# kujason/monopsr

Measured on AMD Instinct MI355X. Metric: instance-crops/sec (fwd+Chamfer), higher is better.
Workload: dtype f32; 1 GPU; BASELINE cfg3: batch=256/GPU synthetic 48x48 crops -> ResNet-101 trunk(block3, os4) + squash/map-decoder/xyz + heads fwd, + 1024-pt nn_distance Chamfer fwd/bwd; batch_per_gpu=256, global_batch=256, points=1024, streams_per_gpu=1

## Files before the change

### include/monopsr_hip.h

```cpp
#ifndef MONOPSR_HIP_H
#define MONOPSR_HIP_H

#include <stddef.h>
#include <stdint.h>

#ifdef __cplusplus
extern "C" {
#endif

typedef void *mpsr_stream_t;
typedef void *mpsr_event_t;

enum {
    MPSR_OK = 0,
    MPSR_ERR_INVALID_ARG = 1,
    MPSR_ERR_HIP = 2,
    MPSR_ERR_WORKSPACE = 3,
    MPSR_ERR_UNSUPPORTED = 4
};

const char *mpsr_last_error(void);
int mpsr_abi_version(void);
uint32_t mpsr_crc32c(uint32_t crc, const void *data, size_t n);

// ... 27 lines not shown
int mpsr_match_cost_grad(int b, int n, int m, const float *xyz1, const float *xyz2, const float *match,
                         float *grad1, float *grad2, mpsr_stream_t stream);


int mpsr_crop_and_resize(const float *image, int nimg, int H, int W, int C, const float *boxes,
                         const int *box_ind, int nb, int ch, int cw, float extrapolation_value, float *out,
                         mpsr_stream_t stream);

int mpsr_resize_bilinear(const float *in, int B, int H, int W, int C, int OH, int OW, int align_corners,
                         float *out, mpsr_stream_t stream);

int mpsr_max_pool(const float *in, int B, int H, int W, int C, int k, int s, int pad_same, float *out,
                  mpsr_stream_t stream);


size_t mpsr_conv2d_scratch_floats(int B, int H, int W, int N);
int mpsr_conv2d_plan(int B, int H, int W, int C, int N, int KH, int KW, int dilation, int *kind,
                     double *executed_flops);
int mpsr_conv2d_nhwc_f32(const float *x, int B, int H, int W, int C, const float *w, const float *bias,
                         const float *residual, float *y, int N, int KH, int KW, int dilation, int relu,
                         int split_k, float *ws, size_t ws_floats, mpsr_stream_t stream);

enum { MPSR_CALL_MATH_INHERIT = 0, MPSR_CALL_MATH_FP32 = 1, MPSR_CALL_MATH_BF16X3 = 2 };
enum { MPSR_CALL_WINOGRAD_INHERIT = 0, MPSR_CALL_WINOGRAD_AUTO = 1, MPSR_CALL_WINOGRAD_OFF = 2,
       MPSR_CALL_WINOGRAD_ACCURATE = 3  };
typedef struct mpsr_conv_opts {
    int32_t math;
    int32_t winograd_policy;
} mpsr_conv_opts;
int mpsr_conv2d_nhwc_f32_ex(const float *x, int B, int H, int W, int C, const float *w, const float *bias,
// ... 304 lines not shown
```

### monopsr_amd/_lib.py

```python
import ctypes
import os

_HERE = os.path.dirname(os.path.abspath(__file__))
LIB_PATH = os.environ.get("MPSR_LIB_PATH") or os.path.join(_HERE, "libmonopsr_hip.so")
ABI_VERSION = 9

_lib = None


class MpsrError(RuntimeError):
    """A libmonopsr_hip.so call returned a non-zero status."""


class InvalidArgumentError(MpsrError, ValueError):
    """Shape/argument check failed -- the analogue of the tf.errors.InvalidArgumentError the reference's
    OP_REQUIRES checks raise (tf_nndistance.cpp:51-58, tf_approxmatch.cpp:152-165)."""


c_f = ctypes.c_void_p
c_i = ctypes.c_int
c_sz = ctypes.c_size_t


class Layer(ctypes.Structure):
# ... 59 lines not shown
    "mpsr_approx_match_temp_floats": (c_sz, [c_i, c_i, c_i]),
    "mpsr_emd_temp_floats": (c_sz, [c_i, c_i, c_i, c_i]),
    "mpsr_emd_loss_temp_floats": (c_sz, [c_i, c_i, c_i, c_i]),
    "mpsr_approx_match": (c_i, [c_i, c_i, c_i, c_f, c_f, c_f, c_f, c_sz, c_f]),
    "mpsr_approx_match_ex": (c_i, [c_i, c_i, c_i, c_f, c_f, c_f, c_f, c_sz, c_i, c_f]),
    "mpsr_emd_loss": (c_i, [c_i, c_i, c_i, c_f, c_f, c_f, c_f, c_f, c_f, c_sz, c_i, c_f]),
    "mpsr_match_cost": (c_i, [c_i, c_i, c_i, c_f, c_f, c_f, c_f, c_f]),
    "mpsr_match_cost_grad": (c_i, [c_i, c_i, c_i, c_f, c_f, c_f, c_f, c_f, c_f]),
    "mpsr_crop_and_resize": (c_i, [c_f, c_i, c_i, c_i, c_i, c_f, c_f, c_i, c_i, c_i, ctypes.c_float, c_f, c_f]),
    "mpsr_resize_bilinear": (c_i, [c_f, c_i, c_i, c_i, c_i, c_i, c_i, c_i, c_f, c_f]),
    "mpsr_max_pool": (c_i, [c_f, c_i, c_i, c_i, c_i, c_i, c_i, c_i, c_f, c_f]),
    "mpsr_conv2d_nhwc_f32": (c_i, [c_f, c_i, c_i, c_i, c_i, c_f, c_f, c_f, c_f, c_i, c_i, c_i, c_i, c_i, c_i, c_f,
                                   c_sz, c_f]),
    "mpsr_conv2d_nhwc_f32_ex": (c_i, [c_f, c_i, c_i, c_i, c_i, c_f, c_f, c_f, c_f, c_i, c_i, c_i, c_i, c_i, c_i, c_f,
                                      c_sz, ctypes.POINTER(ConvOpts), c_f]),
    "mpsr_conv2d_scratch_floats": (c_sz, [c_i, c_i, c_i, c_i]),
    "mpsr_conv2d_plan": (c_i, [c_i] * 8 + [ctypes.POINTER(c_i), ctypes.POINTER(ctypes.c_double)]),
    "mpsr_im2col_root": (c_i, [c_f, c_i, c_i, c_i, c_f, c_i, c_f]),
    "mpsr_conv2d_wgrad_f32": (c_i, [c_f, c_f, c_i, c_i, c_i, c_i, c_i, c_i, c_i, c_i, c_f, c_f, c_f]),
    "mpsr_conv2d_wgrad_scratch_floats": (c_sz, [c_i] * 8),
    "mpsr_conv2d_wgrad_ws_f32": (c_i, [c_f, c_f, c_i, c_i, c_i, c_i, c_i, c_i, c_i, c_i, c_f, c_f, c_f, c_sz, c_f]),
    "mpsr_conv2d_dgrad_pack": (c_i, [c_f, c_i, c_i, c_i, c_i, c_f, c_f]),
    "mpsr_dgrad_pack_table_bytes": (c_sz, [ctypes.POINTER(PackJob), c_i]),
    "mpsr_dgrad_pack_table_build": (c_i, [ctypes.POINTER(PackJob), c_i, ctypes.c_void_p,
                                          ctypes.POINTER(ctypes.c_longlong)]),
    "mpsr_conv2d_dgrad_pack_batch": (c_i, [c_f, ctypes.c_longlong, c_f]),
    "mpsr_act_bias_grad": (c_i, [c_f, c_f, c_f, c_f, ctypes.c_longlong, c_i, c_f]),
    "mpsr_bias_grad": (c_i, [c_f, ctypes.c_longlong, c_i, c_f, c_f]),
    "mpsr_relu_grad": (c_i, [c_f, c_f, c_f, ctypes.c_longlong, c_f]),
    "mpsr_conv2d_relu_masked_f32": (c_i, [c_f, c_i, c_i, c_i, c_i, c_f, c_f, c_f, c_i, c_i, c_i, c_i, c_f, c_sz, c_f]),
# ... 154 lines not shown
```

### monopsr_amd/csrc/conv_mfma.hip

```cpp
#include <atomic>
#include <mutex>
#include <type_traits>

#include "common.h"

namespace {

using f32x16 = __attribute__((ext_vector_type(16))) float;
using f32x4 = __attribute__((ext_vector_type(4))) float;
using bf16x4 = __attribute__((ext_vector_type(4))) __bf16;
using bf16x8 = __attribute__((ext_vector_type(8))) __bf16;

constexpr int MATH_FP32 = 0, MATH_BF16X3 = 1;

constexpr int BK = 32;
constexpr int LDS_STRIDE = BK + 4;
constexpr int MAX_CLS = 9;

using mpsr::FastDiv;
using mpsr::fdiv;
using mpsr::make_fastdiv;

struct PixelClass {
    int y0, h, x0, w;
// ... 935 lines not shown
size_t winograd4_split_floats(int B, int H, int W, int N);
extern std::atomic<int> g_wino4_split;
size_t winograd3_scratch_floats(int C, int N);
bool winograd3_applies(int H, int W, int C, int dilation);
double winograd3_executed_flops(int B, int H, int C, int N, int dilation);
int winograd3_form(int B, int H, int W, int C, int N, int dilation);
int conv3x3_winograd3(const float *x, int B, int H, int W, int C, const float *w, const float *bias, int relu,
                      float *y, int N, int dilation, float *ws, size_t ws_floats, hipStream_t s,
                      const float *mask = nullptr);

bool pointwise_applies(long long M, int K, int N);
int pointwise_override();
int conv1x1_pointwise(const float *x, long long M, int K, const float *w, const float *bias, const float *residual,
                      int relu, float *y, int N, hipStream_t s);

bool thin_input_conv_applies(int B, int H, int W, int C, int N, int KH, int KW, int dilation);
int thin_input_conv(const float *x, int B, int H, int W, const float *w, const float *bias, int relu, float *y, int N,
                    hipStream_t s);

bool fc_rows_applies(long long M, int K, int N);
bool fc_rows_split_applies(long long M, int K, int N, const float *bias, const float *y, const float *ws, size_t ws_floats);
int fc_rows_split(const float *x, long long M, int K, const float *w, const float *bias, int relu, float *y, int N,
                  float *ws, hipStream_t s);
int fc_rows(const float *x, long long M, int K, const float *w, const float *bias, const float *residual, int relu,
            float *y, int N, hipStream_t s);

bool conv2d_takes_fc_rows(int H, int W, long long M, int C, int N, int KH, int KW, int split_k)
{
    const int pw = pointwise_override();
    return H == 1 && W == 1 && KH == 1 && KW == 1 && split_k <= 1 && pw != 0 && cur_math() == MATH_FP32 &&
           g_tile_override.load() < 0 && g_sched_override.load() < 0 && fc_rows_applies(M, C, N);
}

bool conv2d_takes_pointwise(long long M, int C, int N, int KH, int KW, int split_k)
{
    const int pw = pointwise_override();
    if (KH != 1 || KW != 1 || split_k > 1 || pw == 0 || cur_math() != MATH_FP32 || g_tile_override.load() >= 0 ||
        !pointwise_applies(M, C, N))
        return false;
    if (pw > 0) return true;
    if (g_sched_override.load() >= 0 || g_class_override.load() >= 0) return false;
    const long long tiles = ((M + 95) / 96) * ((N + 127) / 128);
    return split_k == 0 && N % 128 == 0 && tiles >= 512;
}

size_t conv_auto_split_floats() { return (size_t)1536 * 64 * 64; }
size_t conv_scratch_floats(long long M, int N)
{
    const size_t slabs = (size_t)1024 * 2 * 96 * 128;
    const size_t counters = (size_t)((M + 63) / 64 + 9) * (size_t)((N + 31) / 32);
    return slabs + counters;
}

int g_auto_split_target = 768;
constexpr int g_auto_split_enough = 768;
constexpr int g_auto_split_min_ksteps = 4;

int auto_split_k(int M, int N, int ksteps, const float *ws, size_t ws_floats)
// ... 79 lines not shown
    const long long M64 = (long long)B * H * W;
    MPSR_REQUIRE(M64 * C * 4 < 0xfffffff0LL && (long long)N * KH * KW * C * 4 < 0xfffffff0LL && M64 < 0x7fffffffLL,
                 "conv2d: tensor exceeds the 4 GiB addressable by one launch; split the batch");
    if (KH == 3 && KW == 3 && dilation == 1 && N <= 4 && C % 32 == 0 && !residual && split_k <= 1 &&
        g_tile_override.load() < 0 && ((uintptr_t)w & 3) == 0)
        return conv3x3_narrow(x, B, H, W, C, w, bias, relu, y, N, stream, 0);
    if (!residual && split_k <= 1 && g_tile_override.load() < 0 && cur_math() == MATH_FP32 &&
        thin_input_conv_applies(B, H, W, C, N, KH, KW, dilation))
        return thin_input_conv(x, B, H, W, w, bias, relu, y, N, stream);
    if (!residual && conv2d_takes_winograd3(B, H, W, C, N, KH, KW, dilation, split_k, ws, ws_floats))
        return conv3x3_winograd3(x, B, H, W, C, w, bias, relu, y, N, dilation, ws, ws_floats, stream);
    {
        const int wc = conv2d_winograd_choice(B, H, W, C, N, KH, KW, dilation, residual != nullptr, split_k, ws, ws_floats);
        if (wc == 2) return conv3x3_winograd4(x, B, H, W, C, w, bias, relu, y, N, ws, ws_floats, stream, 0, 0, nullptr, 0);
        if (wc == 1) return conv3x3_winograd(x, B, H, W, C, w, bias, relu, y, N, ws, ws_floats, stream, dilation);
    }
    if (conv2d_takes_pointwise(M64, C, N, KH, KW, split_k))
        return conv1x1_pointwise(x, M64, C, w, bias, residual, relu, y, N, stream);
    if (conv2d_takes_fc_rows(H, W, M64, C, N, KH, KW, split_k))
        return fc_rows(x, M64, C, w, bias, residual, relu, y, N, stream);
    if (H == 1 && W == 1 && KH == 1 && KW == 1 && !residual && split_k == 0 && pointwise_override() != 0 &&
        cur_math() == MATH_FP32 && g_tile_override.load() < 0 && g_sched_override.load() < 0 &&
        fc_rows_split_applies(M64, C, N, bias, y, ws, ws_floats))
        return fc_rows_split(x, M64, C, w, bias, relu, y, N, ws, stream);
    ConvParams p;
    p.x = x; p.w = w; p.bias = bias; p.residual = residual; p.y = y; p.ws = ws; p.ws_floats = ws ? ws_floats : 0;
    p.M = (int)M64; p.H = H; p.W = W; p.C = C; p.N = N; p.KH = KH; p.KW = KW; p.dil = dilation; p.relu = relu;
    p.xbytes = (unsigned)(M64 * C * 4);
    p.wbytes = (unsigned)((long long)N * KH * KW * C * 4);
    p.cblocks = ceil_div(C, BK);
// ... 125 lines not shown
    if (wc == 1) {
        *kind = 1;
        *executed_flops = 2.0 * (double)B * (H / 2) * (W / 2) * 16.0 * C * N;
        return MPSR_OK;
    }
    if (KH == 3 && KW == 3 && dilation == 1 && N <= 4 && C % 32 == 0) {
        *kind = 2;
        *executed_flops = 2.0 * M * 9.0 * C * N;
        return MPSR_OK;
    }
    if (mpsr::thin_input_conv_applies(B, H, W, C, N, KH, KW, dilation)) {
        *kind = 2;
        *executed_flops = 2.0 * M * 9.0 * C * N;
        return MPSR_OK;
    }
    if (mpsr::conv2d_takes_pointwise((long long)B * H * W, C, N, KH, KW, 0)) {
        *kind = 5;
        *executed_flops = 2.0 * M * C * N;
        return MPSR_OK;
    }
    if (mpsr::conv2d_takes_fc_rows(H, W, (long long)B * H * W, C, N, KH, KW, 0)) {
        *kind = 6;
        *executed_flops = 2.0 * M * C * N;
        return MPSR_OK;
    }
    *kind = 0;
    double taps = (double)KH * KW * H * W;
    if (KH == 3 && KW == 3 && dilation > 1 && H >= 2 * dilation && W >= 2 * dilation) {
        const double ty = 3.0 * H - 2.0 * dilation, tx = 3.0 * W - 2.0 * dilation;
        taps = ty * tx;
// ... 3 lines not shown
}

extern "C" size_t mpsr_conv2d_scratch_floats(int B, int H, int W, int N)
{
    if (B <= 0 || H <= 0 || W <= 0 || N <= 0) return 0;
    size_t n = mpsr::conv_scratch_floats((long long)B * H * W, N);
    if (mpsr::g_wino4_split.load() != 0 && (long long)B * H * W >= 65536 && N % 128 == 0 && H % 4 == 0 && W % 4 == 0)
        n += mpsr::winograd4_split_floats(B, H, W, N) + 64;
    return n;
}

extern "C" int mpsr_conv2d_nhwc_f32(const float *x, int B, int H, int W, int C, const float *w, const float *bias,
                                    const float *residual, float *y, int N, int KH, int KW, int dilation, int relu,
                                    int split_k, float *ws, size_t ws_floats, mpsr_stream_t stream)
{
    return mpsr::conv2d(x, B, H, W, C, w, bias, residual, y, N, KH, KW, dilation, relu, split_k, ws, ws_floats,
                        mpsr::as_stream(stream));
}

extern "C" int mpsr_conv2d_nhwc_f32_ex(const float *x, int B, int H, int W, int C, const float *w, const float *bias,
                                       const float *residual, float *y, int N, int KH, int KW, int dilation, int relu,
                                       int split_k, float *ws, size_t ws_floats, const mpsr_conv_opts *opts,
                                       mpsr_stream_t stream)
{
    if (opts) {
        MPSR_REQUIRE(opts->math >= 0 && opts->math <= MPSR_CALL_MATH_BF16X3, "conv2d: unknown opts.math %d", opts->math);
        MPSR_REQUIRE(opts->winograd_policy >= 0 && opts->winograd_policy <= MPSR_CALL_WINOGRAD_ACCURATE,
                     "conv2d: unknown opts.winograd_policy %d", opts->winograd_policy);
    }
    mpsr::CallOptsGuard guard(opts ? opts->math : 0, opts ? opts->winograd_policy : 0);
    return mpsr::conv2d(x, B, H, W, C, w, bias, residual, y, N, KH, KW, dilation, relu, split_k, ws, ws_floats,
                        mpsr::as_stream(stream));
}

extern "C" int mpsr_conv2d_relu_masked_f32(const float *x, int B, int H, int W, int C, const float *w, const float *mask,
                                           float *y, int N, int KH, int KW, int dilation, float *ws, size_t ws_floats,
                                           mpsr_stream_t stream)
{
    MPSR_REQUIRE(mask, "conv2d_relu_masked: null mask");
    hipStream_t s = mpsr::as_stream(stream);
    if (B > 0 && x && w && y && mpsr::conv2d_takes_winograd3(B, H, W, C, N, KH, KW, dilation, 0, ws, ws_floats))
        return mpsr::conv3x3_winograd3(x, B, H, W, C, w, nullptr, 0, y, N, dilation, ws, ws_floats, s, mask);
    if (int rc = mpsr::conv2d(x, B, H, W, C, w, nullptr, nullptr, y, N, KH, KW, dilation, 0, 0, ws, ws_floats, s)) return rc;
    return mpsr_relu_grad(y, mask, y, (long long)B * H * W * N, stream);
}
// ... 192 lines not shown
```

### monopsr_amd/csrc/network.hip

```cpp
#include <atomic>
#include <vector>

#include "common.h"
#include "wino3_filter.h"

namespace mpsr {
int conv2d(const float *x, int B, int H, int W, int C, const float *w, const float *bias, const float *residual,
           float *y, int N, int KH, int KW, int dilation, int relu, int split_k, float *ws, size_t ws_floats,
           hipStream_t stream);
size_t conv_scratch_floats(long long M, int N);
bool conv2d_takes_winograd4(int B, int H, int W, int C, int N, const float *ws, size_t ws_floats);
int conv3x3_winograd4(const float *x, int B, int H, int W, int C, const float *w, const float *bias, int relu,
                      float *y, int N, float *ws, size_t ws_floats, hipStream_t s, int in_c8, int out_c8, float *part,
                      size_t part_floats);
size_t winograd4_split_floats(int B, int H, int W, int N);
extern std::atomic<int> g_wino4_split;
int winograd3_filter_form(int B, int H, int W, int C, int N, int dilation);
bool conv2d_takes_winograd3(int B, int H, int W, int C, int N, int KH, int KW, int dilation, int split_k, const float *ws,
                            size_t ws_floats);
bool conv2d_takes_pointwise(long long M, int C, int N, int KH, int KW, int split_k);
int conv3x3_narrow(const float *x, int B, int H, int W, int C, const float *w, const float *bias, int relu, float *y,
                   int N, hipStream_t s, int in_c8);
bool conv3x3_narrow_takes_mfma(const float *x, int B, int H, int W, int C, int N, const float *w);
int conv2d_winograd_choice(int B, int H, int W, int C, int N, int KH, int KW, int dilation, bool residual, int split_k,
                           const float *ws, size_t ws_floats);
int resize_bilinear_c8(const float *in, int B, int H, int W, int C, int OH, int OW, int align_corners, float *out,
                       hipStream_t s);
bool upconv_applies(int B, int h, int w, int C, int OH, int OW, int N, int align_corners);
size_t upconv_z_floats(long long Msrc, int N);
size_t upconv_weight_floats(int C, int N);
int conv3x3_upsampled(const float *x, int B, int h, int w, int C, int OH, int OW, int align_corners, const float *g,
                      const float *bias, int relu, float *y, int N, int out_c8, float *z, size_t z_floats, float *ws,
                      size_t ws_floats, hipStream_t s);
}

// ... 28 lines not shown
int run_layer(const float *blob, const mpsr_layer &L, const float *x, int B, int H, int W, const float *residual,
              float *y, int split_k, float *ws, size_t ws_floats, hipStream_t s)
{
    return mpsr::conv2d(x, B, H, W, L.cin, blob + L.w_off, L.b_off >= 0 ? blob + L.b_off : nullptr, residual, y, L.cout,
                        L.kh, L.kw, L.dilation, L.relu, split_k, ws, ws_floats, s);
}

constexpr int kTrunkUnits[3] = {3, 4, 23};

inline size_t cache_floats_of(const mpsr_layer &L)
{
    if (L.kh != 3 || L.kw != 3) return 0;
    return mpsr::align_up((size_t)(L.dilation > 1 ? 25 : 36) * (size_t)L.cout * (size_t)L.cin, 64);
}

struct FilterCache {
    float *base = nullptr;
    size_t floats = 0, used = 0;
    bool valid = false;
    int *tags = nullptr;
    explicit FilterCache(const mpsr_net_opts *o)
    {
        if (o && o->filter_cache && o->filter_cache_floats) {
            base = o->filter_cache;
            floats = o->filter_cache_floats;
            valid = o->filter_cache_valid != 0;
            tags = o->filter_cache_tags;
        }
    }
    float *take(const mpsr_layer &L)
    {
        const size_t need = cache_floats_of(L);
        if (!base || need == 0) return nullptr;
        float *r = used + need <= floats ? base + used : nullptr;
        used += need;
        return r;
    }
    void offer(const float *w, float *slice, const mpsr_layer &L, int layer_index) const
    {
        mpsr::g_filter_cache_slot = mpsr::FilterCacheSlot();
        if (slice) {
            mpsr::g_filter_cache_slot.w = w;
            mpsr::g_filter_cache_slot.u = slice;
            mpsr::g_filter_cache_slot.floats = cache_floats_of(L);
            mpsr::g_filter_cache_slot.ready = valid;
            mpsr::g_filter_cache_slot.tag = tags ? tags + layer_index : nullptr;
        }
    }
};

struct TrunkDims {
// ... 13 lines not shown


extern "C" size_t mpsr_trunk_workspace_bytes(int B, int H, int W)
{
    if (B <= 0 || H <= 0 || W <= 0) return 0;
    const TrunkDims d = trunk_dims(H, W);
    const size_t Mr = (size_t)B * d.OH * d.OW, Mp = (size_t)B * d.PH * d.PW;
    return fbytes(Mr * 160) + fbytes(Mr * 64) + fbytes(Mp * 64) + 3 * fbytes(Mp * 1024) + 2 * fbytes(Mp * 256) +
           fbytes(mpsr::conv_scratch_floats((long long)(Mr > Mp ? Mr : Mp), 1024));
}

extern "C" size_t mpsr_filter_cache_floats(const mpsr_layer *layers, int n_layers)
{
    size_t n = 0;
    if (layers)
        for (int i = 0; i < n_layers; ++i) n += cache_floats_of(layers[i]);
    return n;
}

extern "C" int mpsr_trunk_fwd(const float *img, int B, int H, int W, const float *blob, const mpsr_layer *layers,
                              int n_layers, float *out, void *workspace, size_t workspace_bytes, mpsr_stream_t stream)
{
    return mpsr_trunk_fwd_ex(img, B, H, W, blob, layers, n_layers, out, workspace, workspace_bytes, nullptr, stream);
}

extern "C" int mpsr_trunk_fwd_ex(const float *img, int B, int H, int W, const float *blob, const mpsr_layer *layers,
                                 int n_layers, float *out, void *workspace, size_t workspace_bytes,
                                 const mpsr_net_opts *opts, mpsr_stream_t stream)
{
    MPSR_REQUIRE(B >= 0 && H >= 7 && W >= 7, "trunk_fwd: bad input shape (B=%d H=%d W=%d)", B, H, W);
    if (opts) {
// ... 27 lines not shown
    float *sk = ar.floats(skn);
    if (!ar.ok)
        return mpsr::fail(MPSR_ERR_WORKSPACE, "trunk_fwd: workspace %zu bytes too small (see mpsr_trunk_workspace_bytes)",
                          workspace_bytes);

    int rc;
    struct TailJobGuard {
        ~TailJobGuard()
        {
            mpsr::g_filter_tail_job = mpsr::FilterTailJob();
            mpsr::g_filter_tail_done = mpsr::FilterTailJob();
            mpsr::g_filter_cache_slot = mpsr::FilterCacheSlot();
        }
    } tail_job_guard;
    FilterCache cache(opts);
    if ((rc = mpsr_im2col_root(img, B, H, W, cols, root.cin, stream))) return rc;
    if ((rc = run_layer(blob, root, cols, B, d.OH, d.OW, nullptr, rootout, 0, sk, skn, s))) return rc;
    if ((rc = mpsr_max_pool(rootout, B, d.OH, d.OW, root.cout, 3, 2, 1, pooled, stream))) return rc;

    const float *cur = pooled;
    int cur_c = root.cout;
    int li = 1;
    for (int blk = 0; blk < 3; ++blk) {
        for (int u = 0; u < kTrunkUnits[blk]; ++u) {
            const bool last = (blk == 2 && u == kTrunkUnits[blk] - 1);
            const float *residual = cur;
            if (u == 0) {
                const mpsr_layer &S = layers[li++];
                MPSR_REQUIRE(S.kh == 1 && S.cin == cur_c && !S.relu, "trunk_fwd: record %d is not a shortcut", li - 1);
                if ((rc = run_layer(blob, S, cur, B, d.PH, d.PW, nullptr, scut, 0, sk, skn, s))) return rc;
                residual = scut;
            }
            const mpsr_layer &c1 = layers[li], &c2 = layers[li + 1], &c3 = layers[li + 2];
            li += 3;
            MPSR_REQUIRE(c1.kh == 1 && c1.cin == cur_c && c2.kh == 3 && c2.cin == c1.cout && c3.kh == 1 &&
                             c3.cin == c2.cout && (u == 0 || c3.cout == cur_c),
                         "trunk_fwd: records %d..%d do not form a bottleneck unit", li - 3, li - 1);
            float *dst = last ? out : (cur == ping ? pong : ping);
            float *uslice = cache.take(c2);
            const int c2i = (int)(&c2 - layers);
            const int fform = mpsr::winograd3_filter_form(B, d.PH, d.PW, c2.cin, c2.cout, c2.dilation);
            const bool cached_u = uslice && cache.valid && (!cache.tags || cache.tags[c2i] == fform);
            if (!cached_u &&
                mpsr::conv2d_takes_pointwise((long long)B * d.PH * d.PW, c1.cin, c1.cout, 1, 1, 0) &&
                mpsr::conv2d_takes_winograd3(B, d.PH, d.PW, c2.cin, c2.cout, c2.kh, c2.kw, c2.dilation, 0, sk, skn)) {
                mpsr::g_filter_tail_job.w = blob + c2.w_off;
                mpsr::g_filter_tail_job.u = uslice ? uslice : sk;
                mpsr::g_filter_tail_job.N = c2.cout;
                mpsr::g_filter_tail_job.C = c2.cin;
                mpsr::g_filter_tail_job.form = fform == mpsr::FILTER_FORM_WINO3Z ? 1 : 0;
            }
            if ((rc = run_layer(blob, c1, cur, B, d.PH, d.PW, nullptr, t1, 0, sk, skn, s))) return rc;
            mpsr::g_filter_tail_job = mpsr::FilterTailJob();
            cache.offer(blob + c2.w_off, uslice, c2, c2i);
            rc = run_layer(blob, c2, t1, B, d.PH, d.PW, nullptr, t2, 0, sk, skn, s);
            mpsr::g_filter_cache_slot = mpsr::FilterCacheSlot();
            if (rc) return rc;
            if ((rc = run_layer(blob, c3, t2, B, d.PH, d.PW, residual, dst, 0, sk, skn, s))) return rc;
            cur = dst;
            cur_c = c3.cout;
        }
    }
    return MPSR_OK;
}


namespace {
struct DecoderChoice {
    bool c8, up1, up2, xyz_c8;
};
DecoderChoice decoder_choice(int B, int fh, int fw, int mh, int mw, const mpsr_layer *L, const float *blob, bool feat_map,
                             bool xyz_map, const float *sk, size_t skn)
{
// ... 106 lines not shown
    size_t partn = 0;
    float *partb = nullptr;
    if (ar.ok && mpsr::g_wino4_split.load() != 0 && c2 % 128 == 0 && c3 % 128 == 0 && hh % 4 == 0 && hw % 4 == 0 && mh % 4 == 0 && mw % 4 == 0) {
        const size_t a1 = mpsr::winograd4_split_floats(B, hh, hw, c2), a2 = mpsr::winograd4_split_floats(B, mh, mw, c3);
        partn = (a1 > a2 ? a1 : a2) + 64;
        partb = ar.floats(partn);
        if (!ar.ok) {
            ar.ok = true;
            partb = nullptr;
            partn = 0;
        }
    }
    if (!ar.ok)
        return mpsr::fail(MPSR_ERR_WORKSPACE, "squash_decoder_fwd: workspace %zu bytes too small", workspace_bytes);
    int rc;
    if ((rc = run_layer(blob, L[0], crop_feat, B, fh, fw, nullptr, part, 0, sk, skn, s))) return rc;
    if ((rc = run_layer(blob, L[1], full_feat, B, fh, fw, part, sq, 0, sk, skn, s))) return rc;
    if ((rc = mpsr_max_pool(sq, B, fh, fw, csq, 2, 2, 0, feat_box3d, stream))) return rc;
    if (opts && opts->ready_event) MPSR_CHECK_HIP(hipEventRecord(reinterpret_cast<hipEvent_t>(opts->ready_event), s));
    struct SlotGuard {
        ~SlotGuard() { mpsr::g_filter_cache_slot = mpsr::FilterCacheSlot(); }
    } slot_guard;
    FilterCache cache(opts);
    const DecoderChoice ch = decoder_choice(B, fh, fw, mh, mw, L, blob, feat_map != nullptr, xyz_map != nullptr, sk, skn);
    const bool xyz_c8 = ch.xyz_c8, up1 = ch.up1, up2 = ch.up2, c8 = ch.c8;
    if (c8) {
        auto wino = [&](const mpsr_layer &Lr, const float *x, int H, int W, float *y, int in_c8, int out_c8) {
            cache.offer(blob + Lr.w_off, cache.take(Lr), Lr, (int)(&Lr - L));
            return mpsr::conv3x3_winograd4(x, B, H, W, Lr.cin, blob + Lr.w_off, Lr.b_off >= 0 ? blob + Lr.b_off : nullptr,
                                           Lr.relu, y, Lr.cout, sk, skn, s, in_c8, out_c8, partb, partn);
        };
        auto upconv = [&](const mpsr_layer &Lr, const float *x, int h, int w, int H, int W, float *y, float *z, size_t zn) {
            cache.offer(blob + Lr.w_off, cache.take(Lr), Lr, (int)(&Lr - L));
            return mpsr::conv3x3_upsampled(x, B, h, w, Lr.cin, H, W, 1, blob + Lr.w_off,
                                           Lr.b_off >= 0 ? blob + Lr.b_off : nullptr, Lr.relu, y, Lr.cout, 1, z, zn, sk,
                                           skn, s);
        };
        if (up1) {
// ... 252 lines not shown
```

### monopsr_amd/csrc/wino3_filter.h

```cpp
#pragma once
#include <hip/hip_runtime.h>

namespace mpsr {
namespace f3f {
constexpr int KC = 8, NP = 25;
}

__device__ __forceinline__ void wino3_filter_one(const float *__restrict__ w, int N, int C, float *__restrict__ u, long long i)
{
    const int n = (int)(i / C), c = (int)(i - (long long)n * C);
    double g[3][3];
#pragma unroll
    for (int ky = 0; ky < 3; ++ky)
#pragma unroll
        for (int kx = 0; kx < 3; ++kx) g[ky][kx] = (double)w[(size_t)n * 9 * C + (size_t)(ky * 3 + kx) * C + c];
    auto gcol = [](double a, double b, double c2, double *o) {
        o[0] = a / 2.0;
        o[1] = (a + b + c2) / 2.0;
        o[2] = (a - b + c2) / 6.0;
        o[3] = a / 6.0 + b / 3.0 + c2 * (2.0 / 3.0);
        o[4] = c2;
    };
    double t[5][3];
#pragma unroll
// ... 59 lines not shown
extern thread_local FilterTailJob g_filter_tail_done;

struct FilterCacheSlot {
    const float *w = nullptr;
    float *u = nullptr;
    size_t floats = 0;
    bool ready = false;
    int *tag = nullptr;
    bool holds(int kind)
    {
        const bool ok = ready && (!tag || *tag == kind);
        if (tag) *tag = kind;
        return ok;
    }
};
enum { FILTER_FORM_WINO4 = 1, FILTER_FORM_WINO3 = 2, FILTER_FORM_UPCONV = 3, FILTER_FORM_WINO3Z = 4, FILTER_FORM_WINO2 = 5 };
extern thread_local FilterCacheSlot g_filter_cache_slot;
}
```

### monopsr_amd/csrc/winograd3.hip

```cpp
#include <atomic>
#include <type_traits>

#include "common.h"
#include "wino3_filter.h"
#include "wino3_transforms.h"

namespace {

using f32x16 = __attribute__((ext_vector_type(16))) float;

namespace f3 {
constexpr int MT = 32, NT = 64, KC = 8, NP = 25;
constexpr int APOS = MT * KC;
constexpr int ABUF = NP * APOS;
constexpr int MEXF = NP * 16 * NT;
constexpr int LDSF = MEXF > 2 * ABUF ? MEXF : 2 * ABUF;
constexpr unsigned OOB = 0x80000000u;
}

struct Wino3Params {
    const float *x, *u, *bias;
    float *y;
    int B, H, W, C, N, dil, T;
    int th;
// ... 343 lines not shown
int winograd3_form(int B, int H, int W, int C, int N, int dilation)
{
    const int th = H / (3 * dilation);
    if (th != 1 || !winograd3w_applies(B, H, W, C, N, dilation)) return 0;
    const int form = g_wino3_form.load();
    return (form >= 0 && form <= 2) ? form : 2;
}
int winograd3_filter_form(int B, int H, int W, int C, int N, int dilation)
{
    return winograd3_form(B, H, W, C, N, dilation) == 2 ? FILTER_FORM_WINO3Z : FILTER_FORM_WINO3;
}

thread_local FilterTailJob g_filter_tail_job;
thread_local FilterTailJob g_filter_tail_done;
thread_local FilterCacheSlot g_filter_cache_slot;

size_t winograd3_scratch_floats(int C, int N) { return (size_t)f3::NP * N * C; }

bool winograd3_applies(int H, int W, int C, int dilation)
{
    return dilation >= 1 && H == W && H % (3 * dilation) == 0 && H / (3 * dilation) <= 16 && C % 16 == 0 && C >= 16;
}

long long winograd3_tiles(int B, int H, int dilation)
{
    const int th = H / (3 * dilation);
    return (long long)B * dilation * dilation * th * th;
}
double winograd3_executed_flops(int B, int H, int C, int N, int dilation)
{
// ... 74 lines not shown
```

Baseline: 19280 crops/s.

## Add Strassen 7-multiply pointwise conv kernel with cached filter planes

Adds a 1x1 convolution kernel that applies one level of Strassen over 2x2 blocks of the K and N dimensions. It builds seven combined activation planes in LDS and seven precomputed weight planes, so it issues 7 MFMA products where the plain GEMM issues 8. The weight planes are cached in the trunk and squash filter caches, and half the output quadrants are swapped between waves through LDS before the epilogue. It is on by default when the tile count is large, at the cost of extra adds, LDS traffic, cache memory and looser fp32 accuracy.

```diff
diff --git a/include/monopsr_hip.h b/include/monopsr_hip.h
--- a/include/monopsr_hip.h
+++ b/include/monopsr_hip.h
@@ -65,6 +65,7 @@
                   mpsr_stream_t stream);
 
 
+int mpsr_debug_set_pointwise_strassen(int mode);
 size_t mpsr_conv2d_scratch_floats(int B, int H, int W, int N);
 int mpsr_conv2d_plan(int B, int H, int W, int C, int N, int KH, int KW, int dilation, int *kind,
                      double *executed_flops);
diff --git a/monopsr_amd/_lib.py b/monopsr_amd/_lib.py
--- a/monopsr_amd/_lib.py
+++ b/monopsr_amd/_lib.py
@@ -97,6 +97,7 @@
                                    c_sz, c_f]),
     "mpsr_conv2d_nhwc_f32_ex": (c_i, [c_f, c_i, c_i, c_i, c_i, c_f, c_f, c_f, c_f, c_i, c_i, c_i, c_i, c_i, c_i, c_f,
                                       c_sz, ctypes.POINTER(ConvOpts), c_f]),
+    "mpsr_debug_set_pointwise_strassen": (c_i, [c_i]),
     "mpsr_conv2d_scratch_floats": (c_sz, [c_i, c_i, c_i, c_i]),
     "mpsr_conv2d_plan": (c_i, [c_i] * 8 + [ctypes.POINTER(c_i), ctypes.POINTER(ctypes.c_double)]),
     "mpsr_im2col_root": (c_i, [c_f, c_i, c_i, c_i, c_f, c_i, c_f]),
diff --git a/monopsr_amd/csrc/conv_mfma.hip b/monopsr_amd/csrc/conv_mfma.hip
--- a/monopsr_amd/csrc/conv_mfma.hip
+++ b/monopsr_amd/csrc/conv_mfma.hip
@@ -3,6 +3,7 @@
 #include <type_traits>
 
 #include "common.h"
+#include "wino3_filter.h"
 
 namespace {
 
@@ -973,6 +974,13 @@
 int conv1x1_pointwise(const float *x, long long M, int K, const float *w, const float *bias, const float *residual,
                       int relu, float *y, int N, hipStream_t s);
 
+int pointwise_s7_mode();
+bool pointwise_s7_applies(long long M, int K, int N);
+size_t pointwise_s7_plane_floats(int K, int N);
+int pointwise_s7_fill(const float *w, int K, int N, float *planes, hipStream_t s);
+int conv1x1_pointwise_s7(const float *x, long long M, int K, const float *planes, const float *bias, const float *residual,
+                         int relu, float *y, int N, hipStream_t s);
+
 bool thin_input_conv_applies(int B, int H, int W, int C, int N, int KH, int KW, int dilation);
 int thin_input_conv(const float *x, int B, int H, int W, const float *w, const float *bias, int relu, float *y, int N,
                     hipStream_t s);
@@ -1001,6 +1009,18 @@
     if (g_sched_override.load() >= 0 || g_class_override.load() >= 0) return false;
     const long long tiles = ((M + 95) / 96) * ((N + 127) / 128);
     return split_k == 0 && N % 128 == 0 && tiles >= 512;
+}
+
+bool conv2d_takes_pointwise_s7(long long M, int C, int N, int KH, int KW, int split_k)
+{
+    const int mode = pointwise_s7_mode(), pw = pointwise_override();
+    if (mode == 0 || KH != 1 || KW != 1 || split_k > 1 || pw == 0 || cur_math() != MATH_FP32 || g_tile_override.load() >= 0 ||
+        !pointwise_s7_applies(M, C, N))
+        return false;
+    if (mode == 2) return true;
+    if (pw > 0 || !conv2d_takes_pointwise(M, C, N, KH, KW, split_k)) return false;
+    const long long tiles = ((M + 63) / 64) * (N / 128);
+    return tiles >= 1024;
 }
 
 size_t conv_auto_split_floats() { return (size_t)1536 * 64 * 64; }
@@ -1110,6 +1130,23 @@
         const int wc = conv2d_winograd_choice(B, H, W, C, N, KH, KW, dilation, residual != nullptr, split_k, ws, ws_floats);
         if (wc == 2) return conv3x3_winograd4(x, B, H, W, C, w, bias, relu, y, N, ws, ws_floats, stream, 0, 0, nullptr, 0);
         if (wc == 1) return conv3x3_winograd(x, B, H, W, C, w, bias, relu, y, N, ws, ws_floats, stream, dilation);
+    }
+    if (conv2d_takes_pointwise_s7(M64, C, N, KH, KW, split_k)) {
+        const size_t need = pointwise_s7_plane_floats(C, N);
+        float *planes = nullptr;
+        bool ready = false;
+        if (g_filter_cache_slot.w == w && g_filter_cache_slot.u && g_filter_cache_slot.floats >= need) {
+            planes = g_filter_cache_slot.u;
+            ready = g_filter_cache_slot.holds(FILTER_FORM_PW_S7);
+            g_filter_cache_slot = FilterCacheSlot();
+        } else if (g_conv2d_single_layer && ws && ws_floats >= need && ((uintptr_t)ws & 15) == 0) {
+            planes = ws;
+        }
+        if (planes) {
+            if (!ready)
+                if (int rc = pointwise_s7_fill(w, C, N, planes, stream)) return rc;
+            return conv1x1_pointwise_s7(x, M64, C, planes, bias, residual, relu, y, N, stream);
+        }
     }
     if (conv2d_takes_pointwise(M64, C, N, KH, KW, split_k))
         return conv1x1_pointwise(x, M64, C, w, bias, residual, relu, y, N, stream);
@@ -1265,6 +1302,11 @@
         *executed_flops = 2.0 * M * 9.0 * C * N;
         return MPSR_OK;
     }
+    if (mpsr::conv2d_takes_pointwise_s7((long long)B * H * W, C, N, KH, KW, 0)) {
+        *kind = 5;
+        *executed_flops = 2.0 * M * C * N * 7.0 / 8.0;
+        return MPSR_OK;
+    }
     if (mpsr::conv2d_takes_pointwise((long long)B * H * W, C, N, KH, KW, 0)) {
         *kind = 5;
         *executed_flops = 2.0 * M * C * N;
@@ -1298,6 +1340,10 @@
                                     const float *residual, float *y, int N, int KH, int KW, int dilation, int relu,
                                     int split_k, float *ws, size_t ws_floats, mpsr_stream_t stream)
 {
+    struct SingleLayer {
+        SingleLayer() { mpsr::g_conv2d_single_layer = true; }
+        ~SingleLayer() { mpsr::g_conv2d_single_layer = false; }
+    } single_layer;
     return mpsr::conv2d(x, B, H, W, C, w, bias, residual, y, N, KH, KW, dilation, relu, split_k, ws, ws_floats,
                         mpsr::as_stream(stream));
 }
@@ -1313,6 +1359,10 @@
                      "conv2d: unknown opts.winograd_policy %d", opts->winograd_policy);
     }
     mpsr::CallOptsGuard guard(opts ? opts->math : 0, opts ? opts->winograd_policy : 0);
+    struct SingleLayer {
+        SingleLayer() { mpsr::g_conv2d_single_layer = true; }
+        ~SingleLayer() { mpsr::g_conv2d_single_layer = false; }
+    } single_layer;
     return mpsr::conv2d(x, B, H, W, C, w, bias, residual, y, N, KH, KW, dilation, relu, split_k, ws, ws_floats,
                         mpsr::as_stream(stream));
 }
diff --git a/monopsr_amd/csrc/network.hip b/monopsr_amd/csrc/network.hip
--- a/monopsr_amd/csrc/network.hip
+++ b/monopsr_amd/csrc/network.hip
@@ -19,6 +19,7 @@
 bool conv2d_takes_winograd3(int B, int H, int W, int C, int N, int KH, int KW, int dilation, int split_k, const float *ws,
                             size_t ws_floats);
 bool conv2d_takes_pointwise(long long M, int C, int N, int KH, int KW, int split_k);
+bool conv2d_takes_pointwise_s7(long long M, int C, int N, int KH, int KW, int split_k);
 int conv3x3_narrow(const float *x, int B, int H, int W, int C, const float *w, const float *bias, int relu, float *y,
                    int N, hipStream_t s, int in_c8);
 bool conv3x3_narrow_takes_mfma(const float *x, int B, int H, int W, int C, int N, const float *w);
@@ -77,6 +78,12 @@
     return mpsr::align_up((size_t)(L.dilation > 1 ? 25 : 36) * (size_t)L.cout * (size_t)L.cin, 64);
 }
 
+inline size_t cache_floats_of_1x1(const mpsr_layer &L)
+{
+    if (L.kh != 1 || L.kw != 1 || L.cin < 256 || L.cin > 2048 || L.cin % 64 || L.cout % 128 || L.cout > 2048) return 0;
+    return mpsr::align_up((size_t)7 * (size_t)L.cout * (size_t)L.cin / 4, 64);
+}
+
 struct FilterCache {
     float *base = nullptr;
     size_t floats = 0, used = 0;
@@ -98,6 +105,26 @@
         float *r = used + need <= floats ? base + used : nullptr;
         used += need;
         return r;
+    }
+    size_t base_1x1 = 0, used_1x1 = 0;
+    void layers(const mpsr_layer *L, int n)
+    {
+        for (int i = 0; i < n; ++i) base_1x1 += cache_floats_of(L[i]);
+    }
+    void offer_1x1(const float *w, const mpsr_layer &L, int layer_index, long long M)
+    {
+        const size_t need = cache_floats_of_1x1(L);
+        if (!base || need == 0) return;
+        float *slice = base_1x1 + used_1x1 + need <= floats ? base + base_1x1 + used_1x1 : nullptr;
+        used_1x1 += need;
+        mpsr::g_filter_cache_slot = mpsr::FilterCacheSlot();
+        if (slice && mpsr::conv2d_takes_pointwise_s7(M, L.cin, L.cout, 1, 1, 0)) {
+            mpsr::g_filter_cache_slot.w = w;
+            mpsr::g_filter_cache_slot.u = slice;
+            mpsr::g_filter_cache_slot.floats = need;
+            mpsr::g_filter_cache_slot.ready = valid;
+            mpsr::g_filter_cache_slot.tag = tags ? tags + layer_index : nullptr;
+        }
     }
     void offer(const float *w, float *slice, const mpsr_layer &L, int layer_index) const
     {
@@ -141,7 +168,7 @@
 {
     size_t n = 0;
     if (layers)
-        for (int i = 0; i < n_layers; ++i) n += cache_floats_of(layers[i]);
+        for (int i = 0; i < n_layers; ++i) n += cache_floats_of(layers[i]) + cache_floats_of_1x1(layers[i]);
     return n;
 }
 
@@ -199,6 +226,13 @@
         }
     } tail_job_guard;
     FilterCache cache(opts);
+    cache.layers(layers, n_layers);
+    auto run_1x1 = [&](const mpsr_layer &L1, const float *x, const float *res, float *y) {
+        cache.offer_1x1(blob + L1.w_off, L1, (int)(&L1 - layers), (long long)Mp);
+        const int r = run_layer(blob, L1, x, B, d.PH, d.PW, res, y, 0, sk, skn, s);
+        mpsr::g_filter_cache_slot = mpsr::FilterCacheSlot();
+        return r;
+    };
     if ((rc = mpsr_im2col_root(img, B, H, W, cols, root.cin, stream))) return rc;
     if ((rc = run_layer(blob, root, cols, B, d.OH, d.OW, nullptr, rootout, 0, sk, skn, s))) return rc;
     if ((rc = mpsr_max_pool(rootout, B, d.OH, d.OW, root.cout, 3, 2, 1, pooled, stream))) return rc;
@@ -213,7 +247,7 @@
             if (u == 0) {
                 const mpsr_layer &S = layers[li++];
                 MPSR_REQUIRE(S.kh == 1 && S.cin == cur_c && !S.relu, "trunk_fwd: record %d is not a shortcut", li - 1);
-                if ((rc = run_layer(blob, S, cur, B, d.PH, d.PW, nullptr, scut, 0, sk, skn, s))) return rc;
+                if ((rc = run_1x1(S, cur, nullptr, scut))) return rc;
                 residual = scut;
             }
             const mpsr_layer &c1 = layers[li], &c2 = layers[li + 1], &c3 = layers[li + 2];
@@ -235,13 +269,13 @@
                 mpsr::g_filter_tail_job.C = c2.cin;
                 mpsr::g_filter_tail_job.form = fform == mpsr::FILTER_FORM_WINO3Z ? 1 : 0;
             }
-            if ((rc = run_layer(blob, c1, cur, B, d.PH, d.PW, nullptr, t1, 0, sk, skn, s))) return rc;
+            if ((rc = run_1x1(c1, cur, nullptr, t1))) return rc;
             mpsr::g_filter_tail_job = mpsr::FilterTailJob();
             cache.offer(blob + c2.w_off, uslice, c2, c2i);
             rc = run_layer(blob, c2, t1, B, d.PH, d.PW, nullptr, t2, 0, sk, skn, s);
             mpsr::g_filter_cache_slot = mpsr::FilterCacheSlot();
             if (rc) return rc;
-            if ((rc = run_layer(blob, c3, t2, B, d.PH, d.PW, residual, dst, 0, sk, skn, s))) return rc;
+            if ((rc = run_1x1(c3, t2, residual, dst))) return rc;
             cur = dst;
             cur_c = c3.cout;
         }
@@ -378,14 +412,18 @@
     if (!ar.ok)
         return mpsr::fail(MPSR_ERR_WORKSPACE, "squash_decoder_fwd: workspace %zu bytes too small", workspace_bytes);
     int rc;
-    if ((rc = run_layer(blob, L[0], crop_feat, B, fh, fw, nullptr, part, 0, sk, skn, s))) return rc;
-    if ((rc = run_layer(blob, L[1], full_feat, B, fh, fw, part, sq, 0, sk, skn, s))) return rc;
-    if ((rc = mpsr_max_pool(sq, B, fh, fw, csq, 2, 2, 0, feat_box3d, stream))) return rc;
-    if (opts && opts->ready_event) MPSR_CHECK_HIP(hipEventRecord(reinterpret_cast<hipEvent_t>(opts->ready_event), s));
     struct SlotGuard {
         ~SlotGuard() { mpsr::g_filter_cache_slot = mpsr::FilterCacheSlot(); }
     } slot_guard;
     FilterCache cache(opts);
+    cache.layers(L, n_layers);
+    cache.offer_1x1(blob + L[0].w_off, L[0], 0, (long long)B * fh * fw);
+    if ((rc = run_layer(blob, L[0], crop_feat, B, fh, fw, nullptr, part, 0, sk, skn, s))) return rc;
+    cache.offer_1x1(blob + L[1].w_off, L[1], 1, (long long)B * fh * fw);
+    if ((rc = run_layer(blob, L[1], full_feat, B, fh, fw, part, sq, 0, sk, skn, s))) return rc;
+    mpsr::g_filter_cache_slot = mpsr::FilterCacheSlot();
+    if ((rc = mpsr_max_pool(sq, B, fh, fw, csq, 2, 2, 0, feat_box3d, stream))) return rc;
+    if (opts && opts->ready_event) MPSR_CHECK_HIP(hipEventRecord(reinterpret_cast<hipEvent_t>(opts->ready_event), s));
     const DecoderChoice ch = decoder_choice(B, fh, fw, mh, mw, L, blob, feat_map != nullptr, xyz_map != nullptr, sk, skn);
     const bool xyz_c8 = ch.xyz_c8, up1 = ch.up1, up2 = ch.up2, c8 = ch.c8;
     if (c8) {
diff --git a/monopsr_amd/csrc/pointwise_s7.hip b/monopsr_amd/csrc/pointwise_s7.hip
--- /dev/null
+++ b/monopsr_amd/csrc/pointwise_s7.hip
@@ -0,0 +1,281 @@
+#include <atomic>
+
+#include "common.h"
+#include "wino3_filter.h"
+
+namespace {
+
+using f32x16 = __attribute__((ext_vector_type(16))) float;
+
+namespace s7 {
+constexpr int ROWS = 64, COLS = 128, KS = 32;
+constexpr int PLANE_B = 32 * (KS / 2) * 4;
+constexpr int STAGE_B = 7 * PLANE_B;
+constexpr int XCH_OFF = 2 * STAGE_B;
+constexpr int XCH_B = 4 * 2 * 16 * 64 * 4;
+constexpr int LDS_B = XCH_OFF + XCH_B;
+constexpr unsigned OOB = 0x80000000u;
+}
+
+struct S7Params {
+    const float *x, *planes, *bias, *residual;
+    float *y;
+    int M, N, K, relu;
+    int cblocks, ntiles;
+    unsigned xbytes, pbytes, ybytes;
+    const float *fw;
+    float *fu;
+    int fN, fC, fform;
+};
+
+template <bool RES>
+__global__ __launch_bounds__(256) __attribute__((amdgpu_waves_per_eu(2, 2))) void pw_conv_kernel_s7(const S7Params p)
+{
+    using namespace s7;
+    extern __shared__ __attribute__((aligned(16))) char lds[];
+    const int tid = threadIdx.x, lane = tid & 63;
+    const int wave = __builtin_amdgcn_readfirstlane(tid >> 6);
+    const int wc = wave & 1, kh = wave >> 1;
+    const int nst = p.K / KS;
+    constexpr int STORE_AUX = RES ? 0 : 2;
+
+    const int G = gridDim.x;
+    const int xcd = blockIdx.x & 7, l0 = blockIdx.x >> 3;
+    const int cb = l0 % p.cblocks;
+    const int rgl0 = l0 / p.cblocks, rgstep = (G >> 3) / p.cblocks;
+    const int n_my = (p.ntiles - (int)blockIdx.x + G - 1) / G;
+    auto r0_of = [&](int i) __attribute__((always_inline)) { return ((rgl0 + i * rgstep) * 8 + xcd) * ROWS; };
+    const int n0 = cb * COLS;
+
+    const __amdgpu_buffer_rsrc_t rx = __builtin_amdgcn_make_buffer_rsrc(const_cast<float *>(p.x), 0, (int)p.xbytes, 0x00020000);
+    const __amdgpu_buffer_rsrc_t rp = __builtin_amdgcn_make_buffer_rsrc(const_cast<float *>(p.planes), 0, (int)p.pbytes, 0x00020000);
+    const __amdgpu_buffer_rsrc_t ry = __builtin_amdgcn_make_buffer_rsrc(p.y, 0, (int)p.ybytes, 0x00020000);
+
+    const int prow = tid >> 3, pslot = tid & 7;
+    const unsigned awoff = (unsigned)(prow * 64 + (((pslot >> 1) ^ ((prow >> 2) & 3)) << 4) + (pslot & 1) * 8);
+    float4 stg[2];
+    int lt = 0, ls = 0;
+    auto request_a = [&]() __attribute__((always_inline)) {
+        const int r0 = r0_of(lt);
+        const bool live = lt < n_my;
+#pragma unroll
+        for (int j = 0; j < 2; ++j) {
+            const int row = r0 + 32 * j + prow;
+            const unsigned vo = live && row < p.M ? (unsigned)row * (unsigned)p.K * 4u + (unsigned)pslot * 16u : OOB;
+            stg[j] = __builtin_bit_cast(float4, __builtin_amdgcn_raw_buffer_load_b128(rx, vo, ls * (KS * 4), 0));
+        }
+        ls += 1;
+        if (ls == nst) {
+            ls = 0;
+            lt += 1;
+        }
+    };
+    auto store_a = [&](int buf) __attribute__((always_inline)) {
+        const float4 t0 = stg[0], t1 = stg[1];
+        char *base = lds + buf * STAGE_B + awoff;
+        *reinterpret_cast<float2 *>(base + 0 * PLANE_B) = make_float2(t0.x + t1.z, t0.y + t1.w);
+        *reinterpret_cast<float2 *>(base + 1 * PLANE_B) = make_float2(t1.x + t1.z, t1.y + t1.w);
+        *reinterpret_cast<float2 *>(base + 2 * PLANE_B) = make_float2(t0.x, t0.y);
+        *reinterpret_cast<float2 *>(base + 3 * PLANE_B) = make_float2(t1.z, t1.w);
+        *reinterpret_cast<float2 *>(base + 4 * PLANE_B) = make_float2(t0.x + t0.z, t0.y + t0.w);
+        *reinterpret_cast<float2 *>(base + 5 * PLANE_B) = make_float2(t1.x - t0.x, t1.y - t0.y);
+        *reinterpret_cast<float2 *>(base + 6 * PLANE_B) = make_float2(t0.z - t1.z, t0.w - t1.w);
+    };
+
+    const unsigned pstride = 32u * (unsigned)(p.K / 2) * 4u;
+    const unsigned bvoff = ((unsigned)((n0 + 64 * wc) / 64 * 7 * 32 + (lane & 31)) * (unsigned)(p.K / 2)) * 4u + (unsigned)(lane >> 5) * 16u;
+    float4 fb[7];
+    auto load_b = [&](int i, int stage) __attribute__((always_inline)) {
+        fb[i] = __builtin_bit_cast(float4, __builtin_amdgcn_raw_buffer_load_b128(rp, bvoff, (unsigned)i * pstride + (unsigned)(stage * 64 + kh * 32), 0));
+    };
+
+    const int fr = lane & 31, fh = lane >> 5;
+    const unsigned aroff = (unsigned)(fr * 64 + (((2 * kh + fh) ^ ((fr >> 2) & 3)) << 4));
+    float4 fa[7];
+
+    const int ecol = n0 + 64 * wc + (lane & 31);
+    const float bias0 = p.bias ? p.bias[ecol] : 0.f, bias1 = p.bias ? p.bias[ecol + 32] : 0.f;
+    const float relu_lo = p.relu ? 0.f : -__builtin_inff();
+    const unsigned xw = (unsigned)(XCH_OFF + wave * 8192 + lane * 4), xr = (unsigned)(XCH_OFF + (wave ^ 2) * 8192 + lane * 4);
+
+    request_a();
+#pragma unroll
+    for (int i = 0; i < 7; ++i) load_b(i, 0);
+    store_a(0);
+    request_a();
+    __syncthreads();
+
+    f32x16 acc[7];
+    for (int t = 0; t < n_my; ++t) {
+#pragma unroll
+        for (int i = 0; i < 7; ++i)
+#pragma unroll
+            for (int e = 0; e < 16; ++e) acc[i][e] = 0.f;
+        for (int s = 0; s < nst; ++s) {
+            const int buf = s & 1;
+#pragma unroll
+            for (int i = 0; i < 7; ++i)
+                fa[i] = *reinterpret_cast<const float4 *>(lds + buf * STAGE_B + i * PLANE_B + aroff);
+            store_a(buf ^ 1);
+            request_a();
+            const int bst = s + 1 == nst ? 0 : s + 1;
+            __builtin_amdgcn_sched_barrier(0);
+#pragma unroll
+            for (int i = 0; i < 7; ++i) {
+                acc[i] = __builtin_amdgcn_mfma_f32_32x32x2f32(fa[i].x, fb[i].x, acc[i], 0, 0, 0);
+                acc[i] = __builtin_amdgcn_mfma_f32_32x32x2f32(fa[i].y, fb[i].y, acc[i], 0, 0, 0);
+                acc[i] = __builtin_amdgcn_mfma_f32_32x32x2f32(fa[i].z, fb[i].z, acc[i], 0, 0, 0);
+                acc[i] = __builtin_amdgcn_mfma_f32_32x32x2f32(fa[i].w, fb[i].w, acc[i], 0, 0, 0);
+                load_b(i, bst);
+                __builtin_amdgcn_sched_barrier(0);
+            }
+            __syncthreads();
+        }
+        asm volatile("s_nop 15\n\ts_nop 7"
+                     : "+v"(acc[0]), "+v"(acc[1]), "+v"(acc[2]), "+v"(acc[3]), "+v"(acc[4]), "+v"(acc[5]), "+v"(acc[6]));
+        const int r0 = r0_of(t);
+        unsigned yo[16];
+#pragma unroll
+        for (int e = 0; e < 16; ++e) {
+            const int row = r0 + 32 * kh + (e & 3) + 8 * (e >> 2) + 4 * (lane >> 5);
+            yo[e] = row < p.M ? ((unsigned)row * (unsigned)p.N + (unsigned)ecol) * 4u : OOB;
+        }
+        float res[2][16];
+        if constexpr (RES) {
+            const __amdgpu_buffer_rsrc_t rr =
+                __builtin_amdgcn_make_buffer_rsrc(const_cast<float *>(p.residual), 0, (int)p.ybytes, 0x00020000);
+#pragma unroll
+            for (int c = 0; c < 2; ++c)
+#pragma unroll
+                for (int e = 0; e < 16; ++e)
+                    res[c][e] = __builtin_bit_cast(float, __builtin_amdgcn_raw_buffer_load_b32(rr, yo[e], c * 128, 2));
+        }
+        f32x16 keep[2];
+#pragma unroll
+        for (int e = 0; e < 16; ++e) {
+            const float c11 = ((acc[0][e] + acc[3][e]) - acc[4][e]) + acc[6][e], c12 = acc[2][e] + acc[4][e];
+            const float c21 = acc[1][e] + acc[3][e], c22 = ((acc[0][e] - acc[1][e]) + acc[2][e]) + acc[5][e];
+            keep[0][e] = kh ? c21 : c11;
+            keep[1][e] = kh ? c22 : c12;
+            *reinterpret_cast<float *>(lds + xw + e * 256) = kh ? c11 : c21;
+            *reinterpret_cast<float *>(lds + xw + 4096 + e * 256) = kh ? c12 : c22;
+        }
+        __syncthreads();
+#pragma unroll
+        for (int c = 0; c < 2; ++c)
+#pragma unroll
+            for (int e = 0; e < 16; ++e) {
+                float v = keep[c][e] + *reinterpret_cast<const float *>(lds + xr + c * 4096 + e * 256);
+                v += c ? bias1 : bias0;
+                if constexpr (RES) v += res[c][e];
+                v = fmaxf(v, relu_lo);
+                __builtin_amdgcn_raw_buffer_store_b32(__builtin_bit_cast(unsigned, v), ry, yo[e], c * 128, STORE_AUX);
+            }
+    }
+    if (p.fw) {
+        const long long total = (long long)p.fN * p.fC;
+        for (long long i = (long long)blockIdx.x * 256 + tid; i < total; i += (long long)gridDim.x * 256)
+            if (p.fform) mpsr::wino3z_filter_one(p.fw, p.fN, p.fC, p.fu, i);
+            else mpsr::wino3_filter_one(p.fw, p.fN, p.fC, p.fu, i);
+    }
+}
+
+__global__ __launch_bounds__(256) void pw_s7_filter_kernel(const float *__restrict__ w, int N, int K, float *__restrict__ planes)
+{
+    const int half = K / 2;
+    const long long total = (long long)(N / 64) * 32 * half;
+    const long long i = (long long)blockIdx.x * 256 + threadIdx.x;
+    if (i >= total) return;
+    const int R = (int)(i % half), n = (int)((i / half) % 32), cb = (int)(i / ((long long)half * 32));
+    const int k1 = 4 * (R >> 1) + (R & 1), k2 = k1 + 2;
+    const size_t n1 = (size_t)cb * 64 + n, n2 = n1 + 32;
+    const float b11 = w[n1 * K + k1], b12 = w[n2 * K + k1], b21 = w[n1 * K + k2], b22 = w[n2 * K + k2];
+    float *dst = planes + (((size_t)cb * 7) * 32 + n) * half + R;
+    const size_t ps = (size_t)32 * half;
+    dst[0 * ps] = b11 + b22;
+    dst[1 * ps] = b11;
+    dst[2 * ps] = b12 - b22;
+    dst[3 * ps] = b21 - b11;
+    dst[4 * ps] = b22;
+    dst[5 * ps] = b11 + b12;
+    dst[6 * ps] = b21 + b22;
+}
+
+std::atomic<int> g_pw_s7{1};
+
+}
+
+extern "C" int mpsr_debug_set_pointwise_strassen(int mode)
+{
+    g_pw_s7 = mode < 0 ? 1 : mode > 2 ? 2 : mode;
+    return MPSR_OK;
+}
+
+namespace mpsr {
+
+bool pointwise_applies(long long M, int K, int N);
+
+int pointwise_s7_mode() { return g_pw_s7.load(); }
+
+bool pointwise_s7_applies(long long M, int K, int N)
+{
+    return pointwise_applies(M, K, N) && K >= 256 && K % 64 == 0 && N % 128 == 0 && 7LL * N * K < 0x7f000000LL &&
+           M * N * 4 < 0x7f000000LL;
+}
+
+size_t pointwise_s7_plane_floats(int K, int N) { return (size_t)7 * (size_t)N * (size_t)K / 4; }
+
+int pointwise_s7_fill(const float *w, int K, int N, float *planes, hipStream_t s)
+{
+    const long long total = (long long)(N / 64) * 32 * (K / 2);
+    hipLaunchKernelGGL(pw_s7_filter_kernel, dim3((unsigned)((total + 255) / 256)), dim3(256), 0, s, w, N, K, planes);
+    MPSR_CHECK_LAUNCH("pw_s7_filter_kernel");
+    return MPSR_OK;
+}
+
+int conv1x1_pointwise_s7(const float *x, long long M, int K, const float *planes, const float *bias, const float *residual,
+                         int relu, float *y, int N, hipStream_t s)
+{
+    using namespace s7;
+    MPSR_REQUIRE(pointwise_s7_applies(M, K, N), "conv1x1_pointwise_s7: unsupported shape (M=%lld K=%d N=%d)", M, K, N);
+    S7Params p;
+    p.x = x; p.planes = planes; p.bias = bias; p.residual = residual; p.y = y;
+    p.M = (int)M; p.N = N; p.K = K; p.relu = relu;
+    const int rgroups = (int)((M + ROWS - 1) / ROWS);
+    p.cblocks = N / COLS;
+    p.ntiles = ceil_div(rgroups, 8) * 8 * p.cblocks;
+    p.xbytes = (unsigned)(M * K * 4);
+    p.pbytes = (unsigned)(7LL * N * K);
+    p.ybytes = (unsigned)(M * N * 4);
+    static std::atomic<int> cu_count[64];
+    int dev = 0;
+    MPSR_CHECK_HIP(hipGetDevice(&dev));
+    int cus = dev >= 0 && dev < 64 ? cu_count[dev].load() : 0;
+    if (cus == 0) {
+        int n = 256;
+        MPSR_CHECK_HIP(hipDeviceGetAttribute(&n, hipDeviceAttributeMultiprocessorCount, dev));
+        cus = n > 0 ? n : 256;
+        if (dev >= 0 && dev < 64) cu_count[dev] = cus;
+    }
+    const int unit = 8 * p.cblocks;
+    int grid = 2 * cus / unit * unit;
+    if (grid < unit) grid = unit;
+    if (grid > p.ntiles) grid = p.ntiles;
+    p.fw = g_filter_tail_job.w; p.fu = g_filter_tail_job.u; p.fN = g_filter_tail_job.N; p.fC = g_filter_tail_job.C;
+    p.fform = g_filter_tail_job.form;
+    if (p.fw) g_filter_tail_done = g_filter_tail_job;
+    g_filter_tail_job = FilterTailJob();
+    if (residual) {
+        MPSR_CHECK_HIP(hipFuncSetAttribute(reinterpret_cast<const void *>(pw_conv_kernel_s7<true>),
+                                           hipFuncAttributeMaxDynamicSharedMemorySize, LDS_B));
+        hipLaunchKernelGGL(pw_conv_kernel_s7<true>, dim3(grid), dim3(256), LDS_B, s, p);
+    } else {
+        MPSR_CHECK_HIP(hipFuncSetAttribute(reinterpret_cast<const void *>(pw_conv_kernel_s7<false>),
+                                           hipFuncAttributeMaxDynamicSharedMemorySize, LDS_B));
+        hipLaunchKernelGGL(pw_conv_kernel_s7<false>, dim3(grid), dim3(256), LDS_B, s, p);
+    }
+    MPSR_CHECK_LAUNCH("pw_conv_kernel_s7");
+    return MPSR_OK;
+}
+
+}
diff --git a/monopsr_amd/csrc/wino3_filter.h b/monopsr_amd/csrc/wino3_filter.h
--- a/monopsr_amd/csrc/wino3_filter.h
+++ b/monopsr_amd/csrc/wino3_filter.h
@@ -97,6 +97,8 @@
         return ok;
     }
 };
-enum { FILTER_FORM_WINO4 = 1, FILTER_FORM_WINO3 = 2, FILTER_FORM_UPCONV = 3, FILTER_FORM_WINO3Z = 4, FILTER_FORM_WINO2 = 5 };
+enum { FILTER_FORM_WINO4 = 1, FILTER_FORM_WINO3 = 2, FILTER_FORM_UPCONV = 3, FILTER_FORM_WINO3Z = 4, FILTER_FORM_WINO2 = 5,
+       FILTER_FORM_PW_S7 = 6 };
 extern thread_local FilterCacheSlot g_filter_cache_slot;
+extern thread_local bool g_conv2d_single_layer;
 }
diff --git a/monopsr_amd/csrc/winograd3.hip b/monopsr_amd/csrc/winograd3.hip
--- a/monopsr_amd/csrc/winograd3.hip
+++ b/monopsr_amd/csrc/winograd3.hip
@@ -381,6 +381,7 @@
 thread_local FilterTailJob g_filter_tail_job;
 thread_local FilterTailJob g_filter_tail_done;
 thread_local FilterCacheSlot g_filter_cache_slot;
+thread_local bool g_conv2d_single_layer = false;
 
 size_t winograd3_scratch_floats(int C, int N) { return (size_t)f3::NP * N * C; }
 
```

After: 17880 crops/s. 0.927x the previous value.
